# baudm/parseq

Hardware: NVIDIA H100
Metric: images/sec PARSeq-S 32x128 AR+1refine (higher is better)
Workload: dtype bf16

## Files before the change

parseq_b200/csrc/engine.cu:

```cuda
#include <cuda.h>
#include <cuda_runtime.h>

#include <cmath>
#include <cstdio>
#include <cstdlib>
#include <cstring>
#include <map>
#include <string>
#include <vector>

#include "../../include/parseq_b200.h"
#include "gemm.cuh"
#include "kernels.cuh"
#include "dec_ar.cuh"
#include "dec_ar2.cuh"
#include "gemm_ln.cuh"
#include "mlp_ln.cuh"
#include "attn_wgmma.cuh"

namespace {

constexpr int kMaxHeadClasses = 16384;

thread_local std::string g_last_error;
// ... 177 lines not shown
                               static_cast<int>(pq::dec_ar2_smem_bytes<D, MT, CS>())));
  if constexpr (MT == 1 && CS == 8 && D / 64 <= CS)
    PQ_CUDA(cudaFuncSetAttribute(ar2_kernel<D, MT, CS, true, WIDE>(), cudaFuncAttributeMaxDynamicSharedMemorySize,
                                 static_cast<int>(pq::dec_ar2_smem_bytes<D, MT, CS>())));
  return PARSEQ_OK;
}
template <bool WIDE>
int ar2_set_attributes() {
  PQ_TRY((ar2_attr<192, 1, 8, WIDE>())); PQ_TRY((ar2_attr<192, 2, 8, WIDE>())); PQ_TRY((ar2_attr<384, 1, 8, WIDE>()));
  PQ_TRY((ar2_attr<384, 2, 8, WIDE>())); PQ_TRY((ar2_attr<768, 1, 8, WIDE>()));
  PQ_TRY((ar2_attr<192, 1, 6, WIDE>())); PQ_TRY((ar2_attr<192, 2, 6, WIDE>())); PQ_TRY((ar2_attr<384, 1, 6, WIDE>()));
  PQ_TRY((ar2_attr<384, 2, 6, WIDE>())); PQ_TRY((ar2_attr<768, 1, 6, WIDE>()));
  return PARSEQ_OK;
}

template <int D, int MODE>
int gemm_ln_attr() {
  PQ_CUDA(cudaFuncSetAttribute(pq::gemm_ln_fused_kernel<D, MODE>, cudaFuncAttributeMaxDynamicSharedMemorySize,
                               pq::GemmLnCfg<D, MODE>::kSmemBytes));
  return PARSEQ_OK;
}

template <int D, int CG>
int mlp_ln_attr() {
  PQ_CUDA(cudaFuncSetAttribute(pq::mlp_ln_fused_kernel<D, CG>, cudaFuncAttributeMaxDynamicSharedMemorySize,
                               pq::MlpLnCfg<D, CG>::kSmemBytes));
  return PARSEQ_OK;
}
template <int NK>
int attn_wgmma_attr() {
  PQ_CUDA(cudaFuncSetAttribute(pq::enc_attention_wgmma_kernel<NK>, cudaFuncAttributeMaxDynamicSharedMemorySize,
                               pq::atw_smem_bytes<NK>()));
  return PARSEQ_OK;
}

int init_kernel_attributes() {
  PQ_CUDA(cudaFuncSetAttribute(pq::dec_ar_kernel<192, 1>, cudaFuncAttributeMaxDynamicSharedMemorySize, static_cast<int>(pq::dec_ar_smem_bytes<192>())));
  PQ_CUDA(cudaFuncSetAttribute(pq::dec_ar_kernel<192, 2>, cudaFuncAttributeMaxDynamicSharedMemorySize, static_cast<int>(pq::dec_ar_smem_bytes<192>())));
  PQ_CUDA(cudaFuncSetAttribute(pq::dec_ar_kernel<384, 1>, cudaFuncAttributeMaxDynamicSharedMemorySize, static_cast<int>(pq::dec_ar_smem_bytes<384>())));
  PQ_CUDA(cudaFuncSetAttribute(pq::dec_ar_kernel<384, 2>, cudaFuncAttributeMaxDynamicSharedMemorySize, static_cast<int>(pq::dec_ar_smem_bytes<384>())));
  PQ_CUDA(cudaFuncSetAttribute(pq::dec_ar_kernel<768, 1>, cudaFuncAttributeMaxDynamicSharedMemorySize, static_cast<int>(pq::dec_ar_smem_bytes<768>())));
  PQ_CUDA(cudaFuncSetAttribute(pq::dec_ar_kernel<768, 2>, cudaFuncAttributeMaxDynamicSharedMemorySize, static_cast<int>(pq::dec_ar_smem_bytes<768>())));
  PQ_TRY(ar2_set_attributes<false>());
  PQ_TRY(ar2_set_attributes<true>());
  PQ_CUDA(cudaFuncSetAttribute(pq::dec_ln_head_argmax_kernel<192>, cudaFuncAttributeMaxDynamicSharedMemorySize, 120 * 1024));
  PQ_CUDA(cudaFuncSetAttribute(pq::dec_ln_head_argmax_kernel<384>, cudaFuncAttributeMaxDynamicSharedMemorySize, 160 * 1024));
  PQ_CUDA(cudaFuncSetAttribute(pq::dec_ln_head_argmax_kernel<768>, cudaFuncAttributeMaxDynamicSharedMemorySize, 226 * 1024));
  PQ_TRY((gemm_ln_attr<192, 0>())); PQ_TRY((gemm_ln_attr<384, 0>())); PQ_TRY((gemm_ln_attr<192, 1>()));
  PQ_TRY((gemm_ln_attr<384, 1>())); PQ_TRY((gemm_ln_attr<384, 2>()));
  PQ_TRY((mlp_ln_attr<192, 1>())); PQ_TRY((mlp_ln_attr<384, 1>())); PQ_TRY((mlp_ln_attr<192, 2>())); PQ_TRY((mlp_ln_attr<384, 2>()));
  PQ_TRY((attn_wgmma_attr<128>())); PQ_TRY((attn_wgmma_attr<256>()));
  PQ_TRY((warm_gemm_cfg<pq::EPI_F32, pq::ST_REG>()));
  PQ_TRY((warm_gemm_cfg<pq::EPI_F32_RESID, pq::ST_REG>()));
  PQ_TRY((warm_gemm_cfg<pq::EPI_BF16, pq::ST_REG>()));
  PQ_TRY((warm_gemm_cfg<pq::EPI_BF16, pq::ST_TMA_2D>()));
  PQ_TRY((warm_gemm_cfg<pq::EPI_BF16, pq::ST_TMA_3D>()));
  PQ_TRY((warm_gemm_cfg<pq::EPI_GELU_BF16, pq::ST_REG>()));
  PQ_TRY((warm_gemm_cfg<pq::EPI_GELU_BF16, pq::ST_TMA_2D>()));
  return PARSEQ_OK;
}

int gemm_launch(LaunchOpts& lo, const void* A, long long lda, const void* W, long long ldw, const float* bias, int M, int N,
                int K, int mode, float alpha, const float* resid, long long ldr, int resid_mod, void* out, long long ldo,
                cudaStream_t st, long long blocked_rows = 0) {
// ... 28 lines not shown
  p.num_n_tiles = (N + pq::GEMM_BLOCK_N - 1) / pq::GEMM_BLOCK_N;
  const int tiles = p.num_m_tiles * p.num_n_tiles;
  if (mode == pq::EPI_F32)
    return resid != nullptr ? launch_gemm_cfg<pq::EPI_F32_RESID, pq::ST_REG>(lo, ta, tb, to, p, tiles, st)
                            : launch_gemm_cfg<pq::EPI_F32, pq::ST_REG>(lo, ta, tb, to, p, tiles, st);
  if (mode == pq::EPI_BF16) {
    if (store == pq::ST_TMA_3D) return launch_gemm_cfg<pq::EPI_BF16, pq::ST_TMA_3D>(lo, ta, tb, to, p, tiles, st);
    return store == pq::ST_TMA_2D ? launch_gemm_cfg<pq::EPI_BF16, pq::ST_TMA_2D>(lo, ta, tb, to, p, tiles, st)
                                  : launch_gemm_cfg<pq::EPI_BF16, pq::ST_REG>(lo, ta, tb, to, p, tiles, st);
  }
  return store == pq::ST_TMA_2D ? launch_gemm_cfg<pq::EPI_GELU_BF16, pq::ST_TMA_2D>(lo, ta, tb, to, p, tiles, st)
                                : launch_gemm_cfg<pq::EPI_GELU_BF16, pq::ST_REG>(lo, ta, tb, to, p, tiles, st);
}

bool gemm_ln_supported(int D) { return D == 192 || D == 384; }
template <int D, int MODE>
int launch_gemm_ln(const LaunchOpts& lo, const void* A, long long lda, const void* W, long long ldw, const float* bias, int M, int K, float* x,
                   const float* gamma, const float* beta, float eps, void* xn, cudaStream_t st) {
  using Cfg = pq::GemmLnCfg<D, MODE>;
  static bool attr_set = false;
  if (!attr_set) {
    PQ_TRY((gemm_ln_attr<D, MODE>()));
    attr_set = true;
  }
  CUtensorMap ta, tb;
  PQ_TRY(make_tmap(&ta, A, 2, M, K, lda, pq::GEMM_BLOCK_K, pq::GLN_BLOCK_M));
  PQ_TRY(make_tmap(&tb, W, 2, D, K, ldw, pq::GEMM_BLOCK_K, Cfg::kBox));
  if ((reinterpret_cast<uintptr_t>(x) & 7u) != 0 || (reinterpret_cast<uintptr_t>(xn) & 3u) != 0)
    return fail(PARSEQ_ERR_INVALID_ARG, "gemm_ln: x must be 8-byte and xn 4-byte aligned");
  pq::GemmLnParams p;
  p.M = M; p.K = K; p.bias = bias; p.gamma = gamma; p.beta = beta; p.eps = eps;
  const int tile_m = pq::GLN_BLOCK_M * (MODE == 1 ? 2 : 1);
  p.num_m_tiles = (M + tile_m - 1) / tile_m;
  cudaLaunchConfig_t cfg{};
  cfg.gridDim = dim3(static_cast<unsigned>(p.num_m_tiles * Cfg::kCG));
  cfg.blockDim = dim3(pq::GLN_THREADS);
  cfg.dynamicSmemBytes = Cfg::kSmemBytes;
  cfg.stream = st;
  cudaLaunchAttribute attr[2];
  attr[0].id = cudaLaunchAttributeClusterDimension;
  attr[0].val.clusterDim.x = Cfg::kCG;
  attr[0].val.clusterDim.y = 1;
  attr[0].val.clusterDim.z = 1;
  attr[1].id = cudaLaunchAttributeProgrammaticStreamSerialization;
  attr[1].val.programmaticStreamSerializationAllowed = 1;
  cfg.attrs = attr;
  cfg.numAttrs = (lo.use_pdl && (MODE == 0 || lo.pair_pdl)) ? 2 : 1;
  PQ_CUDA(cudaLaunchKernelEx(&cfg, pq::gemm_ln_fused_kernel<D, MODE>, ta, tb, x, reinterpret_cast<__nv_bfloat16*>(xn), p));
  return PARSEQ_OK;
}
int gemm_ln_launch(LaunchOpts& lo, const void* A, long long lda, const void* W, long long ldw, const float* bias, int M, int D,
                   int K, float* x, const float* gamma, const float* beta, float eps, void* xn, cudaStream_t st) {
  if (M <= 0 || K <= 0) return fail(PARSEQ_ERR_INVALID_ARG, "gemm_ln: empty problem");
  PQ_TRY(ensure_sm_count(lo));
  PQ_TRY(load_driver_api());
  if (D == 384 && (lo.ln_split == 2 || (lo.ln_split == 0 && K >= 768)))
    return launch_gemm_ln<384, 2>(lo, A, lda, W, ldw, bias, M, K, x, gamma, beta, eps, xn, st);
  if (lo.ln_cta_group == 2) {
    if (D == 384) return launch_gemm_ln<384, 1>(lo, A, lda, W, ldw, bias, M, K, x, gamma, beta, eps, xn, st);
    if (D == 192) return launch_gemm_ln<192, 1>(lo, A, lda, W, ldw, bias, M, K, x, gamma, beta, eps, xn, st);
  }
  if (D == 384) return launch_gemm_ln<384, 0>(lo, A, lda, W, ldw, bias, M, K, x, gamma, beta, eps, xn, st);
  if (D == 192) return launch_gemm_ln<192, 0>(lo, A, lda, W, ldw, bias, M, K, x, gamma, beta, eps, xn, st);
  return fail(PARSEQ_ERR_UNSUPPORTED, "gemm_ln: embed_dim must be 192 or 384");
}

template <int D, int CG>
int launch_mlp_ln(const LaunchOpts& lo, const void* xn, const void* W1, const float* b1, const void* W2, const float* b2, int M,
                  float* x, const float* gamma, const float* beta, float eps, void* xn_out, cudaStream_t st) {
  using Cfg = pq::MlpLnCfg<D, CG>;
  static bool attr_set = false;
  if (!attr_set) {
    PQ_TRY((mlp_ln_attr<D, CG>()));
    attr_set = true;
  }
  if ((reinterpret_cast<uintptr_t>(x) & 7u) != 0 || (reinterpret_cast<uintptr_t>(xn_out) & 3u) != 0)
    return fail(PARSEQ_ERR_INVALID_ARG, "mlp_ln: x must be 8-byte and xn_out 4-byte aligned");
  CUtensorMap txn, tw1, tw2;
// ... 1489 lines not shown
```

parseq_b200/csrc/gemm.cuh:

```cuda
#pragma once
#include <cuda.h>
#include "ptx.cuh"

namespace pq {

enum GemmEpilogue : int {
  EPI_F32 = 0,
  EPI_BF16 = 1,
  EPI_GELU_BF16 = 2,
  EPI_F32_RESID = 3,
};
enum GemmStore : int { ST_REG = 0, ST_TMA_2D = 1, ST_TMA_3D = 2 };

struct GemmParams {
  int M, N, K;
  float alpha;
  const float* bias;
  const float* resid;
  long long ldr;
  int resid_mod;
  void* out;
  long long ldo;
  int vec_ok;
  int num_m_tiles, num_n_tiles;
// ... 6 lines not shown
constexpr int GEMM_THREADS = 384;

struct GemmCfg {
  static constexpr int kABytes = GEMM_BLOCK_M * GEMM_BLOCK_K * 2;
  static constexpr int kBBytes = GEMM_BLOCK_N * GEMM_BLOCK_K * 2;
  static constexpr int kStageBytes = kABytes + kBBytes;
  static constexpr int kHalfOutBytes = GEMM_BLOCK_M * 64 * 2;
  static constexpr int kOutBytes = 2 * kHalfOutBytes;
  static constexpr int kStages = 4;
  template <bool STAGING>
  static constexpr int smem_bytes() {
    return kStages * kStageBytes + (STAGING ? 2 * kOutBytes : 0) + 1024  + 256 ;
  }
};
static_assert(GemmCfg::smem_bytes<true>() <= 232448, "shared memory");

template <int N, bool PAIR>
__device__ __forceinline__ void wg_mainloop(float (&acc)[N / 2], uint8_t* smem, int stage_bytes, int a_off, int b_off,
                                            uint64_t* full_bar, uint64_t* empty_bar, int nstages, int num_kb, int& stage,
                                            uint32_t& phase) {
  const bool signal = (threadIdx.x & 127) == 0;
  int prev = -1;
  auto release = [&](int s) {
    if (signal) {
      mbar_arrive(&empty_bar[s]);
      if constexpr (PAIR) mbar_arrive_cluster(mapa_cluster(smem_u32(&empty_bar[s]), cluster_ctarank() ^ 1u));
    }
  };
#pragma unroll 1
  for (int kb = 0; kb < num_kb; ++kb) {
    mbar_wait_mma(&full_bar[stage], phase);
    const uint32_t base = smem_u32(smem + stage * stage_bytes);
    const uint64_t da = make_desc_k_sw128(base + a_off);
    const uint64_t db = make_desc_k_sw128(base + b_off);
    wgmma_fence();
#pragma unroll
    for (int k = 0; k < GEMM_BLOCK_K / 16; ++k)
      wgmma_bf16<N>(acc, da + static_cast<uint64_t>(2 * k), db + static_cast<uint64_t>(2 * k),
                    static_cast<uint32_t>((kb | k) != 0));
    wgmma_commit();
    if (prev >= 0) {
      wgmma_wait<1>();
      release(prev);
    }
    prev = stage;
    if (++stage == nstages) { stage = 0; phase ^= 1u; }
  }
  wgmma_wait<0>();
  wgmma_reg_fence(acc);
  if (prev >= 0) release(prev);
}

__device__ __forceinline__ void ring_advance(int& stage, uint32_t& phase, int n, int nstages) {
  const int s = stage + n;
  phase ^= static_cast<uint32_t>((s / nstages) & 1);
  stage = s % nstages;
}

template <int EPI>
__device__ __forceinline__ float gemm_epi(float v, float b, float alpha) {
  if constexpr (EPI == EPI_GELU_BF16) return gelu_erf(v + b);
  else return (v + b) * alpha;
}

template <int EPI>
__device__ __forceinline__ void gemm_store_pair(const GemmParams& p, int row, int col, float f0, float f1) {
// ... 185 lines not shown
```

parseq_b200/csrc/gemm_ln.cuh:

```cuda
#pragma once
#include "gemm.cuh"

namespace pq {

struct GemmLnParams {
  int M, K;
  const float* bias;
  const float* gamma;
  const float* beta;
  float eps;
  int num_m_tiles;
};

constexpr int GLN_THREADS = 384;
constexpr int GLN_BLOCK_M = 64;

template <int D, int MODE>
struct GemmLnCfg {
  static_assert(MODE >= 0 && MODE <= 2, "MODE");
  static constexpr int kCG = MODE == 0 ? 1 : 2;
  static constexpr int kCols = MODE == 2 ? D / 2 : D;
  static constexpr int kNW = kCols / 2;
  static constexpr int kParts = MODE == 2 ? 4 : 2;
  static constexpr int kLoadRows = MODE == 1 ? D / 2 : kCols;
  static constexpr int kBox = kLoadRows > 256 ? kLoadRows / 2 : kLoadRows;
  static constexpr int kABytes = GLN_BLOCK_M * GEMM_BLOCK_K * 2;
  static constexpr int kBBytes = kCols * GEMM_BLOCK_K * 2;
  static constexpr int kStageBytes = kABytes + kBBytes;
  static constexpr int kParamBytes = 3 * kCols * 4 + 2 * kParts * GLN_BLOCK_M * 4;
  static constexpr int kBarBytes = 256;
  static constexpr int kStagesRaw = (232448 - 1024 - kBarBytes - kParamBytes) / kStageBytes;
  static constexpr int kStages = kStagesRaw > 6 ? 6 : kStagesRaw;
  static constexpr int kSmemBytes = kStages * kStageBytes + kParamBytes + kBarBytes + 1024;
  static_assert(D == 192 || D == 384, "embed_dim");
  static_assert(kNW % 16 == 0 && kNW <= 256, "wgmma N");
  static_assert((kNW * GEMM_BLOCK_K * 2) % 1024 == 0 && (kBox * GEMM_BLOCK_K * 2) % 1024 == 0, "1024-B aligned operand tiles");
  static_assert(kStages >= 3, "pipeline depth");
};

template <int PARTS>
__device__ __forceinline__ float gln_row_total(const float* s_part, int r) {
  float t = s_part[r] + s_part[GLN_BLOCK_M + r];
  if constexpr (PARTS == 4) t += s_part[2 * GLN_BLOCK_M + r] + s_part[3 * GLN_BLOCK_M + r];
  return t;
}

template <int D, int NW, int PARTS, bool SPLIT>
__device__ __forceinline__ void gln_epilogue(float (&acc)[NW / 2], float* __restrict__ x, __nv_bfloat16* __restrict__ xn, int M,
                                             float eps, int m0, int c0, int wg, uint32_t rank, const float* s_bias,
                                             const float* s_gamma, const float* s_beta, float* s_part, uint64_t* stat_bar) {
  constexpr int kNW = NW;
  const int t = threadIdx.x & 127;
  const int lane = t & 31;
  const int lr = (t >> 5) * 16 + (lane >> 2);
  const bool ok_a = m0 + lr < M, ok_b = m0 + lr + 8 < M;
  float* xa = x + static_cast<long long>(m0 + lr) * D + c0 + wg * kNW + 2 * (lane & 3);
  float* xb = xa + 8ll * D;
  const int part = (SPLIT ? static_cast<int>(rank) * 2 : 0) + wg;
  const uint32_t peer = rank ^ 1u;

  float sa = 0.f, sb = 0.f;
#pragma unroll
  for (int i = 0; i < kNW / 8; ++i) {
    const int cl = wg * kNW + i * 8 + 2 * (lane & 3);
    const float b0 = s_bias[cl], b1 = s_bias[cl + 1];
    float2 xo = ok_a ? *reinterpret_cast<const float2*>(xa + i * 8) : make_float2(0.f, 0.f);
    acc[4 * i] = (acc[4 * i] + b0) + xo.x;
    acc[4 * i + 1] = (acc[4 * i + 1] + b1) + xo.y;
    if (ok_a) *reinterpret_cast<float2*>(xa + i * 8) = make_float2(acc[4 * i], acc[4 * i + 1]);
    xo = ok_b ? *reinterpret_cast<const float2*>(xb + i * 8) : make_float2(0.f, 0.f);
    acc[4 * i + 2] = (acc[4 * i + 2] + b0) + xo.x;
    acc[4 * i + 3] = (acc[4 * i + 3] + b1) + xo.y;
    if (ok_b) *reinterpret_cast<float2*>(xb + i * 8) = make_float2(acc[4 * i + 2], acc[4 * i + 3]);
    sa += acc[4 * i] + acc[4 * i + 1];
// ... 5 lines not shown
    if (round == 1) {
      sa = 0.f;
      sb = 0.f;
#pragma unroll
      for (int i = 0; i < kNW / 8; ++i) {
        const float a0 = acc[4 * i] - mean_a, a1 = acc[4 * i + 1] - mean_a;
        const float d0 = acc[4 * i + 2] - mean_b, d1 = acc[4 * i + 3] - mean_b;
        sa += a0 * a0 + a1 * a1;
        sb += d0 * d0 + d1 * d1;
      }
    }
    sa += __shfl_xor_sync(0xffffffffu, sa, 1);
    sa += __shfl_xor_sync(0xffffffffu, sa, 2);
    sb += __shfl_xor_sync(0xffffffffu, sb, 1);
    sb += __shfl_xor_sync(0xffffffffu, sb, 2);
    float* slot = s_part + (round * PARTS + part) * GLN_BLOCK_M;
    if ((lane & 3) == 0) {
      slot[lr] = sa;
      slot[lr + 8] = sb;
      if constexpr (SPLIT) {
        st_cluster_f32(mapa_cluster(smem_u32(slot + lr), peer), sa);
        st_cluster_f32(mapa_cluster(smem_u32(slot + lr + 8), peer), sb);
      }
    }
    if constexpr (SPLIT) {
      mbar_arrive(&stat_bar[round]);
      mbar_arrive_cluster(mapa_cluster(smem_u32(&stat_bar[round]), peer));
      mbar_wait_cluster(&stat_bar[round], 0);
    } else {
      asm volatile("bar.sync 1, 256;" ::: "memory");
    }
    const float* tot = s_part + round * PARTS * GLN_BLOCK_M;
    const float ta = gln_row_total<PARTS>(tot, lr), tb = gln_row_total<PARTS>(tot, lr + 8);
    if (round == 0) {
      mean_a = ta * (1.0f / D);
      mean_b = tb * (1.0f / D);
    } else {
      rstd_a = 1.0f / sqrtf(ta * (1.0f / D) + eps);
      rstd_b = 1.0f / sqrtf(tb * (1.0f / D) + eps);
    }
  }
  uint32_t* na = reinterpret_cast<uint32_t*>(xn + static_cast<long long>(m0 + lr) * D + c0 + wg * kNW + 2 * (lane & 3));
  uint32_t* nb = na + 4ll * D;
#pragma unroll
  for (int i = 0; i < kNW / 8; ++i) {
    const int cl = wg * kNW + i * 8 + 2 * (lane & 3);
    const float g0 = s_gamma[cl], g1 = s_gamma[cl + 1], e0 = s_beta[cl], e1 = s_beta[cl + 1];
    if (ok_a) na[i * 4] = pack_bf16((acc[4 * i] - mean_a) * rstd_a * g0 + e0, (acc[4 * i + 1] - mean_a) * rstd_a * g1 + e1);
    if (ok_b) nb[i * 4] = pack_bf16((acc[4 * i + 2] - mean_b) * rstd_b * g0 + e0, (acc[4 * i + 3] - mean_b) * rstd_b * g1 + e1);
  }
}

template <int D, int MODE>
__global__ void __launch_bounds__(GLN_THREADS, 1)
gemm_ln_fused_kernel(const __grid_constant__ CUtensorMap tmA, const __grid_constant__ CUtensorMap tmB,
                     float* __restrict__ x, __nv_bfloat16* __restrict__ xn, const GemmLnParams p) {
  using Cfg = GemmLnCfg<D, MODE>;
  constexpr int kNW = Cfg::kNW;
  extern __shared__ uint8_t smem_raw[];
  const uint32_t raw_addr = smem_u32(smem_raw);
  const uint32_t pad = ((raw_addr + 1023u) & ~1023u) - raw_addr;
  uint8_t* smem = smem_raw + pad;
  float* s_bias = reinterpret_cast<float*>(smem + Cfg::kStages * Cfg::kStageBytes);
  float* s_gamma = s_bias + Cfg::kCols;
  float* s_beta = s_gamma + Cfg::kCols;
  float* s_part = s_beta + Cfg::kCols;
  uint64_t* full_bar = reinterpret_cast<uint64_t*>(reinterpret_cast<uint8_t*>(s_bias) + Cfg::kParamBytes);
  uint64_t* empty_bar = full_bar + Cfg::kStages;
  uint64_t* stat_bar = empty_bar + Cfg::kStages;

  const uint32_t rank = (MODE != 0) ? cluster_ctarank() : 0u;
  const int cluster = blockIdx.x / Cfg::kCG;
  const int m0 = (MODE == 1) ? cluster * 2 * GLN_BLOCK_M + static_cast<int>(rank) * GLN_BLOCK_M : cluster * GLN_BLOCK_M;
  const int c0 = (MODE == 2) ? static_cast<int>(rank) * Cfg::kCols : 0;
  const int num_kb = (p.K + GEMM_BLOCK_K - 1) / GEMM_BLOCK_K;

  grid_dep_launch();
  if (threadIdx.x == 0) {
    prefetch_tmap(&tmA);
    prefetch_tmap(&tmB);
    for (int s = 0; s < Cfg::kStages; ++s) {
      mbar_init(&full_bar[s], 1);
      mbar_init(&empty_bar[s], MODE == 1 ? 4 : 2);
    }
    mbar_init(&stat_bar[0], 2 * 256);
    mbar_init(&stat_bar[1], 2 * 256);
    fence_mbar_init();
  }
  for (int j = threadIdx.x; j < Cfg::kCols; j += GLN_THREADS) {
    s_bias[j] = (p.bias != nullptr) ? __ldg(p.bias + c0 + j) : 0.0f;
    s_gamma[j] = __ldg(p.gamma + c0 + j);
    s_beta[j] = __ldg(p.beta + c0 + j);
  }
  if constexpr (MODE != 0) cluster_sync_all(); else __syncthreads();
  grid_dep_wait();

  if (threadIdx.x < 128) {
    if (threadIdx.x == 0) {
      int stage = 0;
      uint32_t phase = 0;
      for (int kb = 0; kb < num_kb; ++kb) {
        mbar_wait_mma(&empty_bar[stage], phase ^ 1u);
        uint8_t* sa = smem + stage * Cfg::kStageBytes;
        uint8_t* sb = sa + Cfg::kABytes;
        mbar_expect_tx(&full_bar[stage], Cfg::kStageBytes);
        tma_load_2d(sa, &tmA, &full_bar[stage], kb * GEMM_BLOCK_K, m0);
        if constexpr (MODE == 1) {
          const int r = static_cast<int>(rank);
          tma_load_2d_mcast(sb + r * Cfg::kLoadRows * GEMM_BLOCK_K * 2, &tmB, &full_bar[stage], kb * GEMM_BLOCK_K,
                            r * Cfg::kLoadRows, 0x3);
        } else {
#pragma unroll
          for (int b = 0; b < Cfg::kLoadRows / Cfg::kBox; ++b)
            tma_load_2d(sb + b * Cfg::kBox * GEMM_BLOCK_K * 2, &tmB, &full_bar[stage], kb * GEMM_BLOCK_K, c0 + b * Cfg::kBox);
        }
        if (++stage == Cfg::kStages) { stage = 0; phase ^= 1u; }
      }
    }
    __syncwarp();
  } else {
    const int wg = (threadIdx.x >> 7) - 1;
    float acc[kNW / 2];
#pragma unroll
    for (int i = 0; i < kNW / 2; ++i) acc[i] = 0.0f;
    int stage = 0;
    uint32_t phase = 0;
    wg_mainloop<kNW, MODE == 1>(acc, smem, Cfg::kStageBytes, 0, Cfg::kABytes + wg * kNW * GEMM_BLOCK_K * 2, full_bar,
                                empty_bar, Cfg::kStages, num_kb, stage, phase);
    gln_epilogue<D, kNW, Cfg::kParts, MODE == 2>(acc, x, xn, p.M, p.eps, m0, c0, wg, rank, s_bias, s_gamma, s_beta, s_part,
                                                stat_bar);
  }
  if constexpr (MODE != 0) cluster_sync_all();
}

}
```

parseq_b200/csrc/mlp_ln.cuh:

```cuda
#pragma once
#include "gemm_ln.cuh"

namespace pq {

struct MlpLnParams {
  int M;
  const float* b1;
  const float* b2;
  const float* gamma;
  const float* beta;
  float eps;
  int num_m_tiles;
};

constexpr int MLP_THREADS = 384;

template <int D, int CG>
struct MlpLnCfg {
  static constexpr int kH = 4 * D;
  static constexpr int kKC = D / 64;
  static constexpr int kChunks = kH / 64;
  static constexpr int kW1Rows = 64 / CG;
  static constexpr int kW2Rows = D / 2 / CG;
  static constexpr int kW1Bytes = 64 * 64 * 2;
// ... 144 lines not shown
        mbar_wait_mma(&full_bar[stage], phase);
        if (h == wg) {
          const uint64_t db = make_desc_k_sw128(smem_u32(ring + stage * Cfg::kSlotBytes));
          wgmma_fence();
#pragma unroll
          for (int k = 0; k < 4; ++k)
            wgmma_bf16<D / 2>(acc, da + static_cast<uint64_t>(2 * k), db + static_cast<uint64_t>(2 * k),
                              static_cast<uint32_t>((j | k) != 0));
          wgmma_commit();
          wgmma_wait<0>();
          wgmma_reg_fence(acc);
        }
        release();
      }
    }
    gln_epilogue<D, D / 2, 2, false>(acc, x, xn_out, p.M, p.eps, m0, 0, wg, 0u, s_b2, s_gamma, s_beta, s_part, nullptr);
  }
  if constexpr (CG == 2) cluster_sync_all();
}

}
```

parseq_b200/csrc/ptx.cuh:

```cuda
#pragma once
#include <cuda_bf16.h>
#include <cuda_runtime.h>
#include <stdint.h>

namespace pq {

__device__ __forceinline__ uint32_t smem_u32(const void* p) {
  return static_cast<uint32_t>(__cvta_generic_to_shared(p));
}
__device__ __forceinline__ uint32_t lane_id() { return threadIdx.x & 31u; }

constexpr int ARGMAX_NONE = 0x7fffffff;
__device__ __forceinline__ bool argmax_better(float v, int j, float best, int bi) {
  if (j == ARGMAX_NONE) return false;
  if (bi == ARGMAX_NONE) return true;
  const bool vn = isnan(v), bn = isnan(best);
  if (vn != bn) return vn;
  if (vn || v == best) return j < bi;
  return v > best;
}
__device__ __forceinline__ void argmax_fold(float& best, int& bi, float v, int j) {
  if (argmax_better(v, j, best, bi)) { best = v; bi = j; }
}
__device__ __forceinline__ void argmax_shfl(float& best, int& bi, int lo = 1, int hi = 32) {
// ... 137 lines not shown
__device__ __forceinline__ void tma_reduce_add_2d(const void* tmap, const void* smem_src, int32_t c0, int32_t c1) {
  asm volatile("cp.reduce.async.bulk.tensor.2d.global.shared::cta.add.tile.bulk_group [%0, {%2, %3}], [%1];"
               ::"l"(reinterpret_cast<uint64_t>(tmap)), "r"(smem_u32(smem_src)), "r"(c0), "r"(c1)
               : "memory");
}
__device__ __forceinline__ void bulk_commit_group() { asm volatile("cp.async.bulk.commit_group;" ::: "memory"); }
template <int N>
__device__ __forceinline__ void bulk_wait_group_read() {
  asm volatile("cp.async.bulk.wait_group.read %0;" ::"n"(N) : "memory");
}
template <int N>
__device__ __forceinline__ void bulk_wait_group() {
  asm volatile("cp.async.bulk.wait_group %0;" ::"n"(N) : "memory");
}
__device__ __forceinline__ void fence_proxy_async_smem() { asm volatile("fence.proxy.async.shared::cta;" ::: "memory"); }

__device__ __forceinline__ void tma_load_2d_mcast(void* smem_dst, const void* tmap, uint64_t* bar, int32_t c0, int32_t c1,
                                                  uint16_t cta_mask) {
  asm volatile(
      "cp.async.bulk.tensor.2d.shared::cluster.global.mbarrier::complete_tx::bytes.multicast::cluster [%0], [%1, {%3, %4}], [%2], %5;"
      ::"r"(smem_u32(smem_dst)), "l"(reinterpret_cast<uint64_t>(tmap)), "r"(smem_u32(bar)), "r"(c0), "r"(c1), "h"(cta_mask)
      : "memory");
}
__device__ __forceinline__ void mbar_wait_cluster(uint64_t* bar, uint32_t parity) {
  uint32_t ok = 0;
  long long t0 = clock64();
  uint32_t it = 0;
  while (true) {
    asm volatile(
        "{\n\t.reg .pred p;\n\t"
        "mbarrier.try_wait.parity.acquire.cluster.shared::cta.b64 p, [%1], %2;\n\t"
        "selp.b32 %0, 1, 0, p;\n\t}"
        : "=r"(ok)
        : "r"(smem_u32(bar)), "r"(parity)
        : "memory");
    if (ok) return;
    if (((++it) & 0x3ffu) == 0 && (clock64() - t0) > PQ_SPIN_LIMIT_CYCLES) __trap();
  }
}
__device__ __forceinline__ void st_cluster_f32(uint32_t cluster_addr, float v) {
  asm volatile("st.shared::cluster.f32 [%0], %1;" ::"r"(cluster_addr), "f"(v) : "memory");
}

__device__ __forceinline__ uint64_t make_desc_k_sw128(uint32_t smem_addr) {
  uint64_t d = 0;
  d |= static_cast<uint64_t>((smem_addr >> 4) & 0x3FFFu);
  d |= static_cast<uint64_t>(1u) << 16;
  d |= static_cast<uint64_t>(1024u >> 4) << 32;
  d |= static_cast<uint64_t>(1u) << 62;
  return d;
}
__device__ __forceinline__ void wgmma_fence() { asm volatile("wgmma.fence.sync.aligned;" ::: "memory"); }
__device__ __forceinline__ void wgmma_commit() { asm volatile("wgmma.commit_group.sync.aligned;" ::: "memory"); }
template <int N>
__device__ __forceinline__ void wgmma_wait() { asm volatile("wgmma.wait_group.sync.aligned %0;" ::"n"(N) : "memory"); }
template <int R>
__device__ __forceinline__ void wgmma_reg_fence(float (&d)[R]) {
#pragma unroll
// ... 109 lines not shown
```

Measured before the change: 34220.

## Rework fused GEMM+LayerNorm into persistent full-row tiles with multicast weights

Restructures the fused GEMM+LayerNorm kernel. Each warpgroup now computes a 64-row tile over the full embedding width (one or two N=192 wgmma heads), so row statistics are reduced in registers and the cross-CTA statistics exchange through distributed shared memory and cluster barriers is removed. The kernel becomes persistent: the grid is sized to the number of resident clusters and loops over 128-row groups. With 2-CTA clusters the weight tile is multicast to both CTAs, and an L2 bulk prefetch of the residual rows is issued a few K-blocks before the epilogue. The cost is much higher register pressure (setmaxnreg to 240, up to 192 fp32 accumulators per thread) and a larger B tile per stage, which reduces pipeline depth.

```diff
diff --git a/parseq_b200/csrc/engine.cu b/parseq_b200/csrc/engine.cu
--- a/parseq_b200/csrc/engine.cu
+++ b/parseq_b200/csrc/engine.cu
@@ -215,10 +215,35 @@
   return PARSEQ_OK;
 }
 
-template <int D, int MODE>
-int gemm_ln_attr() {
-  PQ_CUDA(cudaFuncSetAttribute(pq::gemm_ln_fused_kernel<D, MODE>, cudaFuncAttributeMaxDynamicSharedMemorySize,
-                               pq::GemmLnCfg<D, MODE>::kSmemBytes));
+template <int D, int PARTS, int CG>
+int gemm_ln_attr(int* resident_clusters = nullptr) {
+  using Cfg = pq::GemmLnCfg<D, PARTS, CG>;
+  static int resident = 0;
+  if (resident == 0) {
+    PQ_CUDA(cudaFuncSetAttribute(pq::gemm_ln_fused_kernel<D, PARTS, CG>, cudaFuncAttributeMaxDynamicSharedMemorySize,
+                                 Cfg::kSmemBytes));
+    int dev = 0, sms = 0;
+    PQ_CUDA(cudaGetDevice(&dev));
+    PQ_CUDA(cudaDeviceGetAttribute(&sms, cudaDevAttrMultiProcessorCount, dev));
+    resident = sms / CG;
+    if constexpr (CG > 1) {
+      cudaLaunchConfig_t cfg{};
+      cfg.gridDim = dim3(static_cast<unsigned>(sms / CG * CG));
+      cfg.blockDim = dim3(pq::GLN_THREADS);
+      cfg.dynamicSmemBytes = Cfg::kSmemBytes;
+      cudaLaunchAttribute attr[1];
+      attr[0].id = cudaLaunchAttributeClusterDimension;
+      attr[0].val.clusterDim.x = CG;
+      attr[0].val.clusterDim.y = 1;
+      attr[0].val.clusterDim.z = 1;
+      cfg.attrs = attr;
+      cfg.numAttrs = 1;
+      int n = 0;
+      PQ_CUDA(cudaOccupancyMaxActiveClusters(&n, pq::gemm_ln_fused_kernel<D, PARTS, CG>, &cfg));
+      if (n > 0 && n < resident) resident = n;
+    }
+  }
+  if (resident_clusters != nullptr) *resident_clusters = resident;
   return PARSEQ_OK;
 }
 
@@ -247,8 +272,8 @@
   PQ_CUDA(cudaFuncSetAttribute(pq::dec_ln_head_argmax_kernel<192>, cudaFuncAttributeMaxDynamicSharedMemorySize, 120 * 1024));
   PQ_CUDA(cudaFuncSetAttribute(pq::dec_ln_head_argmax_kernel<384>, cudaFuncAttributeMaxDynamicSharedMemorySize, 160 * 1024));
   PQ_CUDA(cudaFuncSetAttribute(pq::dec_ln_head_argmax_kernel<768>, cudaFuncAttributeMaxDynamicSharedMemorySize, 226 * 1024));
-  PQ_TRY((gemm_ln_attr<192, 0>())); PQ_TRY((gemm_ln_attr<384, 0>())); PQ_TRY((gemm_ln_attr<192, 1>()));
-  PQ_TRY((gemm_ln_attr<384, 1>())); PQ_TRY((gemm_ln_attr<384, 2>()));
+  PQ_TRY((gemm_ln_attr<192, 2, 1>())); PQ_TRY((gemm_ln_attr<384, 2, 1>())); PQ_TRY((gemm_ln_attr<192, 2, 2>()));
+  PQ_TRY((gemm_ln_attr<384, 2, 2>())); PQ_TRY((gemm_ln_attr<384, 4, 2>()));
   PQ_TRY((mlp_ln_attr<192, 1>())); PQ_TRY((mlp_ln_attr<384, 1>())); PQ_TRY((mlp_ln_attr<192, 2>())); PQ_TRY((mlp_ln_attr<384, 2>()));
   PQ_TRY((attn_wgmma_attr<128>())); PQ_TRY((attn_wgmma_attr<256>()));
   PQ_TRY((warm_gemm_cfg<pq::EPI_F32, pq::ST_REG>()));
@@ -307,39 +332,37 @@
 }
 
 bool gemm_ln_supported(int D) { return D == 192 || D == 384; }
-template <int D, int MODE>
+template <int D, int PARTS, int CG>
 int launch_gemm_ln(const LaunchOpts& lo, const void* A, long long lda, const void* W, long long ldw, const float* bias, int M, int K, float* x,
                    const float* gamma, const float* beta, float eps, void* xn, cudaStream_t st) {
-  using Cfg = pq::GemmLnCfg<D, MODE>;
-  static bool attr_set = false;
-  if (!attr_set) {
-    PQ_TRY((gemm_ln_attr<D, MODE>()));
-    attr_set = true;
-  }
+  using Cfg = pq::GemmLnCfg<D, PARTS, CG>;
+  int resident = 0;
+  PQ_TRY((gemm_ln_attr<D, PARTS, CG>(&resident)));
   CUtensorMap ta, tb;
-  PQ_TRY(make_tmap(&ta, A, 2, M, K, lda, pq::GEMM_BLOCK_K, pq::GLN_BLOCK_M));
+  PQ_TRY(make_tmap(&ta, A, 2, M, K, lda, pq::GEMM_BLOCK_K, pq::GLN_TILE_M));
   PQ_TRY(make_tmap(&tb, W, 2, D, K, ldw, pq::GEMM_BLOCK_K, Cfg::kBox));
   if ((reinterpret_cast<uintptr_t>(x) & 7u) != 0 || (reinterpret_cast<uintptr_t>(xn) & 3u) != 0)
     return fail(PARSEQ_ERR_INVALID_ARG, "gemm_ln: x must be 8-byte and xn 4-byte aligned");
   pq::GemmLnParams p;
   p.M = M; p.K = K; p.bias = bias; p.gamma = gamma; p.beta = beta; p.eps = eps;
-  const int tile_m = pq::GLN_BLOCK_M * (MODE == 1 ? 2 : 1);
-  p.num_m_tiles = (M + tile_m - 1) / tile_m;
+  p.num_m_tiles = (M + pq::GLN_TILE_M - 1) / pq::GLN_TILE_M;
+  p.num_groups = (p.num_m_tiles + CG - 1) / CG;
+  const int clusters = p.num_groups < resident ? p.num_groups : resident;
   cudaLaunchConfig_t cfg{};
-  cfg.gridDim = dim3(static_cast<unsigned>(p.num_m_tiles * Cfg::kCG));
+  cfg.gridDim = dim3(static_cast<unsigned>(clusters * CG));
   cfg.blockDim = dim3(pq::GLN_THREADS);
   cfg.dynamicSmemBytes = Cfg::kSmemBytes;
   cfg.stream = st;
   cudaLaunchAttribute attr[2];
   attr[0].id = cudaLaunchAttributeClusterDimension;
-  attr[0].val.clusterDim.x = Cfg::kCG;
+  attr[0].val.clusterDim.x = CG;
   attr[0].val.clusterDim.y = 1;
   attr[0].val.clusterDim.z = 1;
   attr[1].id = cudaLaunchAttributeProgrammaticStreamSerialization;
   attr[1].val.programmaticStreamSerializationAllowed = 1;
   cfg.attrs = attr;
-  cfg.numAttrs = (lo.use_pdl && (MODE == 0 || lo.pair_pdl)) ? 2 : 1;
-  PQ_CUDA(cudaLaunchKernelEx(&cfg, pq::gemm_ln_fused_kernel<D, MODE>, ta, tb, x, reinterpret_cast<__nv_bfloat16*>(xn), p));
+  cfg.numAttrs = (lo.use_pdl && (CG == 1 || lo.pair_pdl)) ? 2 : 1;
+  PQ_CUDA(cudaLaunchKernelEx(&cfg, pq::gemm_ln_fused_kernel<D, PARTS, CG>, ta, tb, x, reinterpret_cast<__nv_bfloat16*>(xn), p));
   return PARSEQ_OK;
 }
 int gemm_ln_launch(LaunchOpts& lo, const void* A, long long lda, const void* W, long long ldw, const float* bias, int M, int D,
@@ -348,13 +371,13 @@
   PQ_TRY(ensure_sm_count(lo));
   PQ_TRY(load_driver_api());
   if (D == 384 && (lo.ln_split == 2 || (lo.ln_split == 0 && K >= 768)))
-    return launch_gemm_ln<384, 2>(lo, A, lda, W, ldw, bias, M, K, x, gamma, beta, eps, xn, st);
-  if (lo.ln_cta_group == 2) {
-    if (D == 384) return launch_gemm_ln<384, 1>(lo, A, lda, W, ldw, bias, M, K, x, gamma, beta, eps, xn, st);
-    if (D == 192) return launch_gemm_ln<192, 1>(lo, A, lda, W, ldw, bias, M, K, x, gamma, beta, eps, xn, st);
-  }
-  if (D == 384) return launch_gemm_ln<384, 0>(lo, A, lda, W, ldw, bias, M, K, x, gamma, beta, eps, xn, st);
-  if (D == 192) return launch_gemm_ln<192, 0>(lo, A, lda, W, ldw, bias, M, K, x, gamma, beta, eps, xn, st);
+    return launch_gemm_ln<384, 4, 2>(lo, A, lda, W, ldw, bias, M, K, x, gamma, beta, eps, xn, st);
+  if (lo.ln_cta_group != 1) {
+    if (D == 384) return launch_gemm_ln<384, 2, 2>(lo, A, lda, W, ldw, bias, M, K, x, gamma, beta, eps, xn, st);
+    if (D == 192) return launch_gemm_ln<192, 2, 2>(lo, A, lda, W, ldw, bias, M, K, x, gamma, beta, eps, xn, st);
+  }
+  if (D == 384) return launch_gemm_ln<384, 2, 1>(lo, A, lda, W, ldw, bias, M, K, x, gamma, beta, eps, xn, st);
+  if (D == 192) return launch_gemm_ln<192, 2, 1>(lo, A, lda, W, ldw, bias, M, K, x, gamma, beta, eps, xn, st);
   return fail(PARSEQ_ERR_UNSUPPORTED, "gemm_ln: embed_dim must be 192 or 384");
 }
 
diff --git a/parseq_b200/csrc/gemm.cuh b/parseq_b200/csrc/gemm.cuh
--- a/parseq_b200/csrc/gemm.cuh
+++ b/parseq_b200/csrc/gemm.cuh
@@ -44,42 +44,6 @@
   }
 };
 static_assert(GemmCfg::smem_bytes<true>() <= 232448, "shared memory");
-
-template <int N, bool PAIR>
-__device__ __forceinline__ void wg_mainloop(float (&acc)[N / 2], uint8_t* smem, int stage_bytes, int a_off, int b_off,
-                                            uint64_t* full_bar, uint64_t* empty_bar, int nstages, int num_kb, int& stage,
-                                            uint32_t& phase) {
-  const bool signal = (threadIdx.x & 127) == 0;
-  int prev = -1;
-  auto release = [&](int s) {
-    if (signal) {
-      mbar_arrive(&empty_bar[s]);
-      if constexpr (PAIR) mbar_arrive_cluster(mapa_cluster(smem_u32(&empty_bar[s]), cluster_ctarank() ^ 1u));
-    }
-  };
-#pragma unroll 1
-  for (int kb = 0; kb < num_kb; ++kb) {
-    mbar_wait_mma(&full_bar[stage], phase);
-    const uint32_t base = smem_u32(smem + stage * stage_bytes);
-    const uint64_t da = make_desc_k_sw128(base + a_off);
-    const uint64_t db = make_desc_k_sw128(base + b_off);
-    wgmma_fence();
-#pragma unroll
-    for (int k = 0; k < GEMM_BLOCK_K / 16; ++k)
-      wgmma_bf16<N>(acc, da + static_cast<uint64_t>(2 * k), db + static_cast<uint64_t>(2 * k),
-                    static_cast<uint32_t>((kb | k) != 0));
-    wgmma_commit();
-    if (prev >= 0) {
-      wgmma_wait<1>();
-      release(prev);
-    }
-    prev = stage;
-    if (++stage == nstages) { stage = 0; phase ^= 1u; }
-  }
-  wgmma_wait<0>();
-  wgmma_reg_fence(acc);
-  if (prev >= 0) release(prev);
-}
 
 __device__ __forceinline__ void ring_advance(int& stage, uint32_t& phase, int n, int nstages) {
   const int s = stage + n;
diff --git a/parseq_b200/csrc/gemm_ln.cuh b/parseq_b200/csrc/gemm_ln.cuh
--- a/parseq_b200/csrc/gemm_ln.cuh
+++ b/parseq_b200/csrc/gemm_ln.cuh
@@ -10,54 +10,52 @@
   const float* beta;
   float eps;
   int num_m_tiles;
+  int num_groups;
 };
 
 constexpr int GLN_THREADS = 384;
 constexpr int GLN_BLOCK_M = 64;
-
-template <int D, int MODE>
+constexpr int GLN_TILE_M = 128;
+constexpr int GLN_PREFETCH_CHUNK = 32768;
+constexpr int GLN_PREFETCH_LEAD_KB = 3;
+
+template <int D, int PARTS, int CG>
 struct GemmLnCfg {
-  static_assert(MODE >= 0 && MODE <= 2, "MODE");
-  static constexpr int kCG = MODE == 0 ? 1 : 2;
-  static constexpr int kCols = MODE == 2 ? D / 2 : D;
-  static constexpr int kNW = kCols / 2;
-  static constexpr int kParts = MODE == 2 ? 4 : 2;
-  static constexpr int kLoadRows = MODE == 1 ? D / 2 : kCols;
-  static constexpr int kBox = kLoadRows > 256 ? kLoadRows / 2 : kLoadRows;
-  static constexpr int kABytes = GLN_BLOCK_M * GEMM_BLOCK_K * 2;
-  static constexpr int kBBytes = kCols * GEMM_BLOCK_K * 2;
+  static constexpr int kNH = D / 192;
+  static constexpr int kLoadRows = D / CG;
+  static constexpr int kBox = kLoadRows > 192 ? 192 : kLoadRows;
+  static constexpr int kABytes = GLN_TILE_M * GEMM_BLOCK_K * 2;
+  static constexpr int kBBytes = D * GEMM_BLOCK_K * 2;
   static constexpr int kStageBytes = kABytes + kBBytes;
-  static constexpr int kParamBytes = 3 * kCols * 4 + 2 * kParts * GLN_BLOCK_M * 4;
+  static constexpr int kParamBytes = 3 * D * 4;
   static constexpr int kBarBytes = 256;
   static constexpr int kStagesRaw = (232448 - 1024 - kBarBytes - kParamBytes) / kStageBytes;
   static constexpr int kStages = kStagesRaw > 6 ? 6 : kStagesRaw;
   static constexpr int kSmemBytes = kStages * kStageBytes + kParamBytes + kBarBytes + 1024;
   static_assert(D == 192 || D == 384, "embed_dim");
-  static_assert(kNW % 16 == 0 && kNW <= 256, "wgmma N");
-  static_assert((kNW * GEMM_BLOCK_K * 2) % 1024 == 0 && (kBox * GEMM_BLOCK_K * 2) % 1024 == 0, "1024-B aligned operand tiles");
+  static_assert(PARTS == 2 || (PARTS == 4 && D == 384), "statistics grouping");
+  static_assert(CG == 1 || CG == 2, "cluster size");
+  static_assert(kLoadRows % kBox == 0 && (kBox * GEMM_BLOCK_K * 2) % 1024 == 0, "1024-B aligned operand boxes");
   static_assert(kStages >= 3, "pipeline depth");
 };
 
-template <int PARTS>
-__device__ __forceinline__ float gln_row_total(const float* s_part, int r) {
-  float t = s_part[r] + s_part[GLN_BLOCK_M + r];
-  if constexpr (PARTS == 4) t += s_part[2 * GLN_BLOCK_M + r] + s_part[3 * GLN_BLOCK_M + r];
-  return t;
-}
-
-template <int D, int NW, int PARTS, bool SPLIT>
-__device__ __forceinline__ void gln_epilogue(float (&acc)[NW / 2], float* __restrict__ x, __nv_bfloat16* __restrict__ xn, int M,
-                                             float eps, int m0, int c0, int wg, uint32_t rank, const float* s_bias,
-                                             const float* s_gamma, const float* s_beta, float* s_part, uint64_t* stat_bar) {
-  constexpr int kNW = NW;
+__device__ __forceinline__ void prefetch_rows_l2(const void* src, uint32_t bytes) {
+  const char* p = static_cast<const char*>(src);
+  for (uint32_t off = 0; off < bytes; off += GLN_PREFETCH_CHUNK)
+    prefetch_l2_bulk(p + off, bytes - off < GLN_PREFETCH_CHUNK ? bytes - off : GLN_PREFETCH_CHUNK);
+}
+
+template <int D>
+__device__ __forceinline__ void gln_epilogue(float (&acc)[D / 4], float* __restrict__ x, __nv_bfloat16* __restrict__ xn, int M,
+                                             float eps, int m0, int wg, const float* s_bias, const float* s_gamma,
+                                             const float* s_beta, float* s_part) {
+  constexpr int kNW = D / 2;
   const int t = threadIdx.x & 127;
   const int lane = t & 31;
   const int lr = (t >> 5) * 16 + (lane >> 2);
   const bool ok_a = m0 + lr < M, ok_b = m0 + lr + 8 < M;
-  float* xa = x + static_cast<long long>(m0 + lr) * D + c0 + wg * kNW + 2 * (lane & 3);
+  float* xa = x + static_cast<long long>(m0 + lr) * D + wg * kNW + 2 * (lane & 3);
   float* xb = xa + 8ll * D;
-  const int part = (SPLIT ? static_cast<int>(rank) * 2 : 0) + wg;
-  const uint32_t peer = rank ^ 1u;
 
   float sa = 0.f, sb = 0.f;
 #pragma unroll
@@ -93,24 +91,14 @@
     sa += __shfl_xor_sync(0xffffffffu, sa, 2);
     sb += __shfl_xor_sync(0xffffffffu, sb, 1);
     sb += __shfl_xor_sync(0xffffffffu, sb, 2);
-    float* slot = s_part + (round * PARTS + part) * GLN_BLOCK_M;
+    float* slot = s_part + (round * 2 + wg) * GLN_BLOCK_M;
     if ((lane & 3) == 0) {
       slot[lr] = sa;
       slot[lr + 8] = sb;
-      if constexpr (SPLIT) {
-        st_cluster_f32(mapa_cluster(smem_u32(slot + lr), peer), sa);
-        st_cluster_f32(mapa_cluster(smem_u32(slot + lr + 8), peer), sb);
-      }
-    }
-    if constexpr (SPLIT) {
-      mbar_arrive(&stat_bar[round]);
-      mbar_arrive_cluster(mapa_cluster(smem_u32(&stat_bar[round]), peer));
-      mbar_wait_cluster(&stat_bar[round], 0);
-    } else {
-      asm volatile("bar.sync 1, 256;" ::: "memory");
-    }
-    const float* tot = s_part + round * PARTS * GLN_BLOCK_M;
-    const float ta = gln_row_total<PARTS>(tot, lr), tb = gln_row_total<PARTS>(tot, lr + 8);
+    }
+    asm volatile("bar.sync 1, 256;" ::: "memory");
+    const float* tot = s_part + round * 2 * GLN_BLOCK_M;
+    const float ta = tot[lr] + tot[GLN_BLOCK_M + lr], tb = tot[lr + 8] + tot[GLN_BLOCK_M + lr + 8];
     if (round == 0) {
       mean_a = ta * (1.0f / D);
       mean_b = tb * (1.0f / D);
@@ -119,7 +107,7 @@
       rstd_b = 1.0f / sqrtf(tb * (1.0f / D) + eps);
     }
   }
-  uint32_t* na = reinterpret_cast<uint32_t*>(xn + static_cast<long long>(m0 + lr) * D + c0 + wg * kNW + 2 * (lane & 3));
+  uint32_t* na = reinterpret_cast<uint32_t*>(xn + static_cast<long long>(m0 + lr) * D + wg * kNW + 2 * (lane & 3));
   uint32_t* nb = na + 4ll * D;
 #pragma unroll
   for (int i = 0; i < kNW / 8; ++i) {
@@ -130,29 +118,38 @@
   }
 }
 
-template <int D, int MODE>
+__device__ __forceinline__ float gln_quad_sum(float s) {
+  s += __shfl_xor_sync(0xffffffffu, s, 1);
+  s += __shfl_xor_sync(0xffffffffu, s, 2);
+  return s;
+}
+template <int PARTS>
+__device__ __forceinline__ float gln_parts_total(const float (&s)[PARTS]) {
+  if constexpr (PARTS == 4) return (s[0] + s[1]) + (s[2] + s[3]);
+  else return s[0] + s[1];
+}
+
+template <int D, int PARTS, int CG>
 __global__ void __launch_bounds__(GLN_THREADS, 1)
 gemm_ln_fused_kernel(const __grid_constant__ CUtensorMap tmA, const __grid_constant__ CUtensorMap tmB,
                      float* __restrict__ x, __nv_bfloat16* __restrict__ xn, const GemmLnParams p) {
-  using Cfg = GemmLnCfg<D, MODE>;
-  constexpr int kNW = Cfg::kNW;
+  using Cfg = GemmLnCfg<D, PARTS, CG>;
+  constexpr int kNH = Cfg::kNH;
   extern __shared__ uint8_t smem_raw[];
   const uint32_t raw_addr = smem_u32(smem_raw);
   const uint32_t pad = ((raw_addr + 1023u) & ~1023u) - raw_addr;
   uint8_t* smem = smem_raw + pad;
   float* s_bias = reinterpret_cast<float*>(smem + Cfg::kStages * Cfg::kStageBytes);
-  float* s_gamma = s_bias + Cfg::kCols;
-  float* s_beta = s_gamma + Cfg::kCols;
-  float* s_part = s_beta + Cfg::kCols;
+  float* s_gamma = s_bias + D;
+  float* s_beta = s_gamma + D;
   uint64_t* full_bar = reinterpret_cast<uint64_t*>(reinterpret_cast<uint8_t*>(s_bias) + Cfg::kParamBytes);
   uint64_t* empty_bar = full_bar + Cfg::kStages;
-  uint64_t* stat_bar = empty_bar + Cfg::kStages;
-
-  const uint32_t rank = (MODE != 0) ? cluster_ctarank() : 0u;
-  const int cluster = blockIdx.x / Cfg::kCG;
-  const int m0 = (MODE == 1) ? cluster * 2 * GLN_BLOCK_M + static_cast<int>(rank) * GLN_BLOCK_M : cluster * GLN_BLOCK_M;
-  const int c0 = (MODE == 2) ? static_cast<int>(rank) * Cfg::kCols : 0;
+
+  const uint32_t rank = (CG == 2) ? cluster_ctarank() : 0u;
+  const int cluster = static_cast<int>(blockIdx.x) / CG;
+  const int num_clusters = static_cast<int>(gridDim.x) / CG;
   const int num_kb = (p.K + GEMM_BLOCK_K - 1) / GEMM_BLOCK_K;
+  auto tile_row = [&](int grp) { return (grp * CG + static_cast<int>(rank)) * GLN_TILE_M; };
 
   grid_dep_launch();
   if (threadIdx.x == 0) {
@@ -160,56 +157,154 @@
     prefetch_tmap(&tmB);
     for (int s = 0; s < Cfg::kStages; ++s) {
       mbar_init(&full_bar[s], 1);
-      mbar_init(&empty_bar[s], MODE == 1 ? 4 : 2);
-    }
-    mbar_init(&stat_bar[0], 2 * 256);
-    mbar_init(&stat_bar[1], 2 * 256);
+      mbar_init(&empty_bar[s], 2 * CG);
+    }
     fence_mbar_init();
   }
-  for (int j = threadIdx.x; j < Cfg::kCols; j += GLN_THREADS) {
-    s_bias[j] = (p.bias != nullptr) ? __ldg(p.bias + c0 + j) : 0.0f;
-    s_gamma[j] = __ldg(p.gamma + c0 + j);
-    s_beta[j] = __ldg(p.beta + c0 + j);
-  }
-  if constexpr (MODE != 0) cluster_sync_all(); else __syncthreads();
+  for (int j = threadIdx.x; j < D; j += GLN_THREADS) {
+    s_bias[j] = (p.bias != nullptr) ? __ldg(p.bias + j) : 0.0f;
+    s_gamma[j] = __ldg(p.gamma + j);
+    s_beta[j] = __ldg(p.beta + j);
+  }
+  if constexpr (CG == 2) cluster_sync_all(); else __syncthreads();
   grid_dep_wait();
 
   if (threadIdx.x < 128) {
+    setmaxnreg_dec<24>();
     if (threadIdx.x == 0) {
       int stage = 0;
       uint32_t phase = 0;
-      for (int kb = 0; kb < num_kb; ++kb) {
-        mbar_wait_mma(&empty_bar[stage], phase ^ 1u);
-        uint8_t* sa = smem + stage * Cfg::kStageBytes;
-        uint8_t* sb = sa + Cfg::kABytes;
-        mbar_expect_tx(&full_bar[stage], Cfg::kStageBytes);
-        tma_load_2d(sa, &tmA, &full_bar[stage], kb * GEMM_BLOCK_K, m0);
-        if constexpr (MODE == 1) {
-          const int r = static_cast<int>(rank);
-          tma_load_2d_mcast(sb + r * Cfg::kLoadRows * GEMM_BLOCK_K * 2, &tmB, &full_bar[stage], kb * GEMM_BLOCK_K,
-                            r * Cfg::kLoadRows, 0x3);
-        } else {
-#pragma unroll
-          for (int b = 0; b < Cfg::kLoadRows / Cfg::kBox; ++b)
-            tma_load_2d(sb + b * Cfg::kBox * GEMM_BLOCK_K * 2, &tmB, &full_bar[stage], kb * GEMM_BLOCK_K, c0 + b * Cfg::kBox);
+      for (int grp = cluster; grp < p.num_groups; grp += num_clusters) {
+        const int m0 = tile_row(grp);
+        for (int kb = 0; kb < num_kb; ++kb) {
+          mbar_wait_mma(&empty_bar[stage], phase ^ 1u);
+          uint8_t* sa = smem + stage * Cfg::kStageBytes;
+          uint8_t* sb = sa + Cfg::kABytes + rank * Cfg::kLoadRows * GEMM_BLOCK_K * 2;
+          mbar_expect_tx(&full_bar[stage], Cfg::kStageBytes);
+          tma_load_2d(sa, &tmA, &full_bar[stage], kb * GEMM_BLOCK_K, m0);
+#pragma unroll
+          for (int b = 0; b < Cfg::kLoadRows / Cfg::kBox; ++b) {
+            const int r0 = static_cast<int>(rank) * Cfg::kLoadRows + b * Cfg::kBox;
+            if constexpr (CG == 2)
+              tma_load_2d_mcast(sb + b * Cfg::kBox * GEMM_BLOCK_K * 2, &tmB, &full_bar[stage], kb * GEMM_BLOCK_K, r0, 0x3);
+            else
+              tma_load_2d(sb + b * Cfg::kBox * GEMM_BLOCK_K * 2, &tmB, &full_bar[stage], kb * GEMM_BLOCK_K, r0);
+          }
+          if (++stage == Cfg::kStages) { stage = 0; phase ^= 1u; }
         }
-        if (++stage == Cfg::kStages) { stage = 0; phase ^= 1u; }
-      }
-    }
-    __syncwarp();
+      }
+    }
   } else {
+    setmaxnreg_inc<240>();
     const int wg = (threadIdx.x >> 7) - 1;
-    float acc[kNW / 2];
-#pragma unroll
-    for (int i = 0; i < kNW / 2; ++i) acc[i] = 0.0f;
+    const int t = threadIdx.x & 127;
+    const int lane = t & 31;
+    const int lr = (t >> 5) * 16 + (lane >> 2);
+    const bool leader = t == 0;
+    auto release = [&](int s) {
+      if (leader) {
+        mbar_arrive(&empty_bar[s]);
+        if constexpr (CG == 2) mbar_arrive_cluster(mapa_cluster(smem_u32(&empty_bar[s]), rank ^ 1u));
+      }
+    };
     int stage = 0;
     uint32_t phase = 0;
-    wg_mainloop<kNW, MODE == 1>(acc, smem, Cfg::kStageBytes, 0, Cfg::kABytes + wg * kNW * GEMM_BLOCK_K * 2, full_bar,
-                                empty_bar, Cfg::kStages, num_kb, stage, phase);
-    gln_epilogue<D, kNW, Cfg::kParts, MODE == 2>(acc, x, xn, p.M, p.eps, m0, c0, wg, rank, s_bias, s_gamma, s_beta, s_part,
-                                                stat_bar);
-  }
-  if constexpr (MODE != 0) cluster_sync_all();
-}
-
-}
+#pragma unroll 1
+    for (int grp = cluster; grp < p.num_groups; grp += num_clusters) {
+      float acc[kNH][96];
+#pragma unroll
+      for (int h = 0; h < kNH; ++h)
+#pragma unroll
+        for (int i = 0; i < 96; ++i) acc[h][i] = 0.0f;
+      int prev = -1;
+#pragma unroll 1
+      for (int kb = 0; kb < num_kb; ++kb) {
+        if (leader && kb == (num_kb > GLN_PREFETCH_LEAD_KB ? num_kb - GLN_PREFETCH_LEAD_KB : 0) &&
+            (reinterpret_cast<uintptr_t>(x) & 15u) == 0) {
+          const int r0 = tile_row(grp) + wg * GLN_BLOCK_M;
+          if (r0 < p.M) {
+            const int rows = p.M - r0 < GLN_BLOCK_M ? p.M - r0 : GLN_BLOCK_M;
+            prefetch_rows_l2(x + static_cast<long long>(r0) * D, static_cast<uint32_t>(rows) * D * 4u);
+          }
+        }
+        mbar_wait_mma(&full_bar[stage], phase);
+        const uint32_t base = smem_u32(smem + stage * Cfg::kStageBytes);
+        const uint64_t da = make_desc_k_sw128(base + wg * GLN_BLOCK_M * GEMM_BLOCK_K * 2);
+        wgmma_fence();
+#pragma unroll
+        for (int k = 0; k < GEMM_BLOCK_K / 16; ++k)
+#pragma unroll
+          for (int h = 0; h < kNH; ++h)
+            wgmma_bf16<192>(acc[h], da + static_cast<uint64_t>(2 * k),
+                            make_desc_k_sw128(base + Cfg::kABytes + h * 192 * GEMM_BLOCK_K * 2) + static_cast<uint64_t>(2 * k),
+                            static_cast<uint32_t>((kb | k) != 0));
+        wgmma_commit();
+        if (prev >= 0) {
+          wgmma_wait<1>();
+          release(prev);
+        }
+        prev = stage;
+        if (++stage == Cfg::kStages) { stage = 0; phase ^= 1u; }
+      }
+      wgmma_wait<0>();
+#pragma unroll
+      for (int h = 0; h < kNH; ++h) wgmma_reg_fence(acc[h]);
+      release(prev);
+
+      constexpr int kG = D / 8;
+      constexpr int kGP = kG / PARTS;
+      const int ra = tile_row(grp) + wg * GLN_BLOCK_M + lr;
+      const bool ok_a = ra < p.M, ok_b = ra + 8 < p.M;
+      float* xa = x + static_cast<long long>(ra) * D + 2 * (lane & 3);
+      float* xb = xa + 8ll * D;
+      float sa[PARTS], sb[PARTS];
+#pragma unroll
+      for (int g = 0; g < kG; ++g) {
+        float* v = &acc[g / 24][4 * (g % 24)];
+        const int col = g * 8 + 2 * (lane & 3);
+        const float b0 = s_bias[col], b1 = s_bias[col + 1];
+        float2 xo = ok_a ? *reinterpret_cast<const float2*>(xa + g * 8) : make_float2(0.f, 0.f);
+        v[0] = (v[0] + b0) + xo.x;
+        v[1] = (v[1] + b1) + xo.y;
+        if (ok_a) *reinterpret_cast<float2*>(xa + g * 8) = make_float2(v[0], v[1]);
+        xo = ok_b ? *reinterpret_cast<const float2*>(xb + g * 8) : make_float2(0.f, 0.f);
+        v[2] = (v[2] + b0) + xo.x;
+        v[3] = (v[3] + b1) + xo.y;
+        if (ok_b) *reinterpret_cast<float2*>(xb + g * 8) = make_float2(v[2], v[3]);
+        if (g % kGP == 0) { sa[g / kGP] = 0.f; sb[g / kGP] = 0.f; }
+        sa[g / kGP] += v[0] + v[1];
+        sb[g / kGP] += v[2] + v[3];
+      }
+#pragma unroll
+      for (int q = 0; q < PARTS; ++q) { sa[q] = gln_quad_sum(sa[q]); sb[q] = gln_quad_sum(sb[q]); }
+      const float mean_a = gln_parts_total<PARTS>(sa) * (1.0f / D);
+      const float mean_b = gln_parts_total<PARTS>(sb) * (1.0f / D);
+#pragma unroll
+      for (int g = 0; g < kG; ++g) {
+        const float* v = &acc[g / 24][4 * (g % 24)];
+        const float a0 = v[0] - mean_a, a1 = v[1] - mean_a;
+        const float d0 = v[2] - mean_b, d1 = v[3] - mean_b;
+        if (g % kGP == 0) { sa[g / kGP] = 0.f; sb[g / kGP] = 0.f; }
+        sa[g / kGP] += a0 * a0 + a1 * a1;
+        sb[g / kGP] += d0 * d0 + d1 * d1;
+      }
+#pragma unroll
+      for (int q = 0; q < PARTS; ++q) { sa[q] = gln_quad_sum(sa[q]); sb[q] = gln_quad_sum(sb[q]); }
+      const float rstd_a = 1.0f / sqrtf(gln_parts_total<PARTS>(sa) * (1.0f / D) + p.eps);
+      const float rstd_b = 1.0f / sqrtf(gln_parts_total<PARTS>(sb) * (1.0f / D) + p.eps);
+      uint32_t* na = reinterpret_cast<uint32_t*>(xn + static_cast<long long>(ra) * D + 2 * (lane & 3));
+      uint32_t* nb = na + 4ll * D;
+#pragma unroll
+      for (int g = 0; g < kG; ++g) {
+        const float* v = &acc[g / 24][4 * (g % 24)];
+        const int col = g * 8 + 2 * (lane & 3);
+        const float g0 = s_gamma[col], g1 = s_gamma[col + 1], e0 = s_beta[col], e1 = s_beta[col + 1];
+        if (ok_a) na[g * 4] = pack_bf16((v[0] - mean_a) * rstd_a * g0 + e0, (v[1] - mean_a) * rstd_a * g1 + e1);
+        if (ok_b) nb[g * 4] = pack_bf16((v[2] - mean_b) * rstd_b * g0 + e0, (v[3] - mean_b) * rstd_b * g1 + e1);
+      }
+    }
+  }
+  if constexpr (CG == 2) cluster_sync_all();
+}
+
+}
diff --git a/parseq_b200/csrc/mlp_ln.cuh b/parseq_b200/csrc/mlp_ln.cuh
--- a/parseq_b200/csrc/mlp_ln.cuh
+++ b/parseq_b200/csrc/mlp_ln.cuh
@@ -182,7 +182,7 @@
         release();
       }
     }
-    gln_epilogue<D, D / 2, 2, false>(acc, x, xn_out, p.M, p.eps, m0, 0, wg, 0u, s_b2, s_gamma, s_beta, s_part, nullptr);
+    gln_epilogue<D>(acc, x, xn_out, p.M, p.eps, m0, wg, s_b2, s_gamma, s_beta, s_part);
   }
   if constexpr (CG == 2) cluster_sync_all();
 }
diff --git a/parseq_b200/csrc/ptx.cuh b/parseq_b200/csrc/ptx.cuh
--- a/parseq_b200/csrc/ptx.cuh
+++ b/parseq_b200/csrc/ptx.cuh
@@ -175,6 +175,9 @@
   asm volatile("cp.async.bulk.wait_group %0;" ::"n"(N) : "memory");
 }
 __device__ __forceinline__ void fence_proxy_async_smem() { asm volatile("fence.proxy.async.shared::cta;" ::: "memory"); }
+__device__ __forceinline__ void prefetch_l2_bulk(const void* gsrc, uint32_t bytes) {
+  asm volatile("cp.async.bulk.prefetch.L2.global [%0], %1;" ::"l"(reinterpret_cast<uint64_t>(gsrc)), "r"(bytes) : "memory");
+}
 
 __device__ __forceinline__ void tma_load_2d_mcast(void* smem_dst, const void* tmap, uint64_t* bar, int32_t c0, int32_t c1,
                                                   uint16_t cta_mask) {
@@ -183,26 +186,6 @@
       ::"r"(smem_u32(smem_dst)), "l"(reinterpret_cast<uint64_t>(tmap)), "r"(smem_u32(bar)), "r"(c0), "r"(c1), "h"(cta_mask)
       : "memory");
 }
-__device__ __forceinline__ void mbar_wait_cluster(uint64_t* bar, uint32_t parity) {
-  uint32_t ok = 0;
-  long long t0 = clock64();
-  uint32_t it = 0;
-  while (true) {
-    asm volatile(
-        "{\n\t.reg .pred p;\n\t"
-        "mbarrier.try_wait.parity.acquire.cluster.shared::cta.b64 p, [%1], %2;\n\t"
-        "selp.b32 %0, 1, 0, p;\n\t}"
-        : "=r"(ok)
-        : "r"(smem_u32(bar)), "r"(parity)
-        : "memory");
-    if (ok) return;
-    if (((++it) & 0x3ffu) == 0 && (clock64() - t0) > PQ_SPIN_LIMIT_CYCLES) __trap();
-  }
-}
-__device__ __forceinline__ void st_cluster_f32(uint32_t cluster_addr, float v) {
-  asm volatile("st.shared::cluster.f32 [%0], %1;" ::"r"(cluster_addr), "f"(v) : "memory");
-}
-
 __device__ __forceinline__ uint64_t make_desc_k_sw128(uint32_t smem_addr) {
   uint64_t d = 0;
   d |= static_cast<uint64_t>((smem_addr >> 4) & 0x3FFFu);
```

Result: faster. 36420, median of 6 (+6.4%).
